# mosure/bevy_gaussian_splatting

Measured on NVIDIA H100. Metric: rendered Msplats/sec @1080p, 6M-gaussian cloud, higher is better.
Workload: dtype f32 (f16-packed inputs)

## Files before the change

bevy_gaussian_splatting_b200/csrc/project.cu:

```cuda
#include "project_math.cuh"
#include "launch.cuh"

namespace bgs {

__constant__ float c_shc[16] = {
    0.28209479177387814f, -0.4886025119029199f, 0.4886025119029199f, -0.4886025119029199f,
    1.0925484305920792f, -1.0925484305920792f, 0.31539156525252005f, -1.0925484305920792f,
    0.5462742152960396f, -0.5900435899266435f, 2.890611442640554f, -0.4570457994644658f,
    0.3731763325901154f, -0.4570457994644658f, 1.445305721320277f, -0.5900435899266435f};

__device__ __forceinline__ void normalize3(const float a[3], float out[3]) {
    const float inv = rsqrtf((a[0] * a[0] + a[1] * a[1]) + a[2] * a[2]);
    out[0] = a[0] * inv; out[1] = a[1] * inv; out[2] = a[2] * inv;
}
__device__ __forceinline__ float dot3(const float a[3], const float b[3]) {
    return (a[0] * b[0] + a[1] * b[1]) + a[2] * b[2];
}
__device__ __forceinline__ float srgb_to_linear(float v) {
    if (v <= 0.04045f) return v * (1.0f / 12.92f);
    return __powf((v + 0.055f) * (1.0f / 1.055f), 2.4f);
}
__device__ __forceinline__ uint32_t pack_bbox(float lo, float hi) {
    return (uint32_t)(int)lo | ((uint32_t)(int)hi << 16);
}
constexpr uint32_t BBOX_EMPTY = 1u;

__device__ __forceinline__ void make_bbox(float cx, float cy, float hx, float hy, int Wi, int Hi,
                                          uint32_t& bx, uint32_t& by) {
    bx = BBOX_EMPTY; by = BBOX_EMPTY;
    if (!(hx >= 0.0f) || !(hy >= 0.0f) || !(cx == cx) || !(cy == cy)) return;
    const float sx = hx * 1.0e-3f + 1.0e-2f, sy = hy * 1.0e-3f + 1.0e-2f;
    float x0 = ceilf((cx - hx) - (0.5f + sx));
    float x1 = floorf((cx + hx) - (0.5f - sx));
    float y0 = ceilf((cy - hy) - (0.5f + sy));
    float y1 = floorf((cy + hy) - (0.5f - sy));
    if (!(x0 <= x1) || !(y0 <= y1)) return;
    x0 = fmaxf(x0, 0.0f); y0 = fmaxf(y0, 0.0f);
    x1 = fminf(x1, (float)(Wi - 1)); y1 = fminf(y1, (float)(Hi - 1));
    if (!(x0 <= x1) || !(y0 <= y1)) return;
    bx = pack_bbox(x0, x1); by = pack_bbox(y0, y1);
}

__device__ __forceinline__ void cp_async16(uint4* dst_shared, const uint4* src) {
    asm volatile("cp.async.cg.shared.global [%0], [%1], 16;" ::"r"((uint32_t)__cvta_generic_to_shared(dst_shared)), "l"(src)
                 : "memory");
}
__device__ __forceinline__ void cp_async_commit() { asm volatile("cp.async.commit_group;" ::: "memory"); }
template <int N>
__device__ __forceinline__ void cp_async_wait() { asm volatile("cp.async.wait_group %0;" ::"n"(N) : "memory"); }

template <int CH>
__device__ __forceinline__ int stage_slot(int p, int g) {
    static_assert(CH % 8 == 0 || CH == 4, "blocks of 4 or a multiple of 8 chunks");
    if constexpr (CH == 4) return p ^ ((g >> 1) & 3);
    else return p ^ (g & 7);
}

template <int CH, int NP>
__device__ __forceinline__ void gather_blocks(const uint4* __restrict__ blocks, uint32_t id, uint32_t n_valid,
                                              uint4* stage, int lane) {
    static_assert(32 % NP == 0 && NP <= CH, "NP lanes per block");
#pragma unroll
    for (int k = 0; k < NP; ++k) {
        const int g = (32 * k + lane) / NP, p = lane % NP;
        const uint32_t gid = __shfl_sync(0xFFFFFFFFu, id, g);
        if ((uint32_t)g < n_valid) cp_async16(stage + g * CH + stage_slot<CH>(p, g), blocks + (size_t)gid * CH + p);
    }
}

template <bool F16, uint32_t D>
struct Attr;
template <uint32_t D>
struct Attr<false, D> {
    static constexpr CloudLayout L = CloudLayout::F32;
    static constexpr int CH = chunks(L, D), GEO = 4;
    __device__ static float4 load(const uint4* stage, int g, float* sh, float q[4], float so[4], bool need_sh, uint32_t&) {
        auto piece = [&](int p) {
            const uint4 v = stage[g * CH + stage_slot<CH>(p, g)];
            return make_float4(__uint_as_float(v.x), __uint_as_float(v.y), __uint_as_float(v.z), __uint_as_float(v.w));
        };
        const float4 p = piece(POS_CHUNK), r = piece(SECOND_CHUNK), s = piece(SO_CHUNK);
        q[0] = r.x; q[1] = r.y; q[2] = r.z; q[3] = r.w;
        so[0] = s.x; so[1] = s.y; so[2] = s.z; so[3] = s.w;
        if (need_sh) {
#pragma unroll
            for (int i = 0; i < (int)sh_chunks(L, D); ++i) {
                const float4 v = piece(sh_first(L) + i);
                sh[4 * i] = v.x; sh[4 * i + 1] = v.y; sh[4 * i + 2] = v.z; sh[4 * i + 3] = v.w;
            }
        }
        return p;
    }
};
template <uint32_t D>
struct Attr<true, D> {
    static constexpr CloudLayout L = CloudLayout::F16;
    static constexpr int CH = chunks(L, D), GEO = 2;
    static constexpr int FULL = (int)sh_floats(D) / 8;
    __device__ static float4 load(const uint4* stage, int g, float* sh, float q[4], float so[4], bool need_sh,
                                  uint32_t& op_bits) {
        auto piece = [&](int p) { return stage[g * CH + stage_slot<CH>(p, g)]; };
        const uint4 pw = piece(POS_CHUNK), w = piece(SECOND_CHUNK);
        op_bits = w.w & 0xFFFFu;
        second_lanes(w.x, w.y, q);
        second_lanes(w.z, w.w, so);
        if (need_sh) {
#pragma unroll
            for (int i = 0; i < FULL; ++i) {
                const uint4 v = piece(sh_first(L) + i);
                sh[8 * i] = half_lo(v.x); sh[8 * i + 1] = half_hi(v.x); sh[8 * i + 2] = half_lo(v.y); sh[8 * i + 3] = half_hi(v.y);
                sh[8 * i + 4] = half_lo(v.z); sh[8 * i + 5] = half_hi(v.z); sh[8 * i + 6] = half_lo(v.w); sh[8 * i + 7] = half_hi(v.w);
            }
            if constexpr (sh_floats(D) % 8 != 0) {
                const uint4 v = piece(sh_first(L) + FULL);
                sh[8 * FULL] = half_lo(v.x); sh[8 * FULL + 1] = half_hi(v.x);
                sh[8 * FULL + 2] = half_lo(v.y); sh[8 * FULL + 3] = half_hi(v.y);
            }
        }
        return make_float4(__uint_as_float(pw.x), __uint_as_float(pw.y), __uint_as_float(pw.z), __uint_as_float(pw.w));
    }
};

template <CloudLayout L, uint32_t D>
__device__ __forceinline__ void repack_chunk(const CloudPlanes<const uint4>& planes, uint32_t n, uint4* __restrict__ blocks,
                                             const uint4* __restrict__ tt) {
    constexpr uint32_t CH = chunks(L, D);
    const size_t i = (size_t)blockIdx.x * blockDim.x + threadIdx.x;
    if (i >= (size_t)n * CH) return;
    const uint4* src = planes.unit<L, D>((uint32_t)(i % CH), i / CH, tt);
    blocks[i] = src ? __ldg(src) : make_uint4(0u, 0u, 0u, 0u);
}
template <CloudLayout L, uint32_t D>
__global__ void repack_kernel(CloudPlanes<const uint4> planes, uint32_t n, uint4* __restrict__ blocks) {
    repack_chunk<L, D>(planes, n, blocks, nullptr);
}
__global__ void repack_4d_kernel(CloudPlanes<const uint4> planes, uint32_t n, uint4* __restrict__ blocks,
                                 const uint4* __restrict__ tt) {
    repack_chunk<CloudLayout::F32x4D, SH_DEGREE_MAX>(planes, n, blocks, tt);
}
void launch_repack(CloudLayout layout, uint32_t sh_degree, const void* sh, const void* rot, const void* so, const void* tt,
                   uint32_t n, CloudView cloud, cudaStream_t stream) {
    const CloudPlanes<const uint4> planes{reinterpret_cast<const uint4*>(cloud.pos), static_cast<const uint4*>(sh),
                                          static_cast<const uint4*>(rot), static_cast<const uint4*>(so)};
    const uint32_t grid = (uint32_t)(((size_t)n * cloud.chunks + 255) / 256);
    with_layout_degree(layout, sh_degree, [&](auto L, auto D) {
        if constexpr (is_4d(decltype(L)::value))
            repack_4d_kernel<<<grid, 256, 0, stream>>>(planes, n, cloud.blocks, static_cast<const uint4*>(tt));
        else
            repack_kernel<decltype(L)::value, decltype(D)::value><<<grid, 256, 0, stream>>>(planes, n, cloud.blocks);
    });
}

__global__ void depth_range_kernel(const float4* __restrict__ pos, uint32_t n, const uint32_t* __restrict__ sorted_payload,
                                   const uint32_t* __restrict__ slot_ids ,
                                   FrameCounters* __restrict__ ctr, FrameConsts fc) {
    if (threadIdx.x != 0 || blockIdx.x != 0 || n < 2u) return;
    const uint32_t n_vis = ctr->n_vis, n_sorted = ctr->n_sort;
    auto id_at = [&](uint32_t i) { const uint32_t p = sorted_payload[i]; return slot_ids ? slot_ids[p] : p; };
    uint32_t first, last;
    if (n_sorted == n) {
        first = id_at(1u); last = id_at(n - 1u);
    } else {
        const uint32_t cmin = 0xFFFFFFFFu - ctr->culled_min_inv, cmax = ctr->culled_max_p1 - 1u;
        first = n_vis >= 2u ? id_at(1u) : cmin;
        last = (n - n_vis) >= 1u ? cmax : id_at(n - 1u);
    }
    auto dist = [&](uint32_t id) {
        const float4 p = pos[id];
        float pw[4];
        mat4_point(fc.model, p.x, p.y, p.z, pw);
        return sqrtf(cam_dist2(fc, pw));
    };
    ctr->depth_min = dist(last);
    ctr->depth_max = dist(first);
}

__device__ __forceinline__ float adaptive_cutoff(float opacity) {
    const float a = 9.0f + 2.0f * det_ln(opacity);
    return sqrtf(a > 0.000001f ? a : 0.000001f);
}
__global__ void cutoff_table_kernel(float* __restrict__ tab) {
    const uint32_t h = blockIdx.x * blockDim.x + threadIdx.x;
    if (h < 65536u) tab[h] = adaptive_cutoff(__half2float(__ushort_as_half((unsigned short)h)));
}
void launch_cutoff_table(float* tab, cudaStream_t stream) { cutoff_table_kernel<<<256, 256, 0, stream>>>(tab); }

template <bool F16>
__device__ __forceinline__ float splat_cutoff(const FrameConsts& fc, float opacity, const float* __restrict__ cutoff_tab,
                                              uint32_t op_bits) {
    if (!fc.adaptive) return 3.0f;
    if constexpr (F16) return __ldg(cutoff_tab + op_bits);
    else return adaptive_cutoff(opacity);
}

__device__ __forceinline__ void rotation_rows(const float q[4], float Rm[3][3]) {
    const float qr = q[0], x = q[1], y = q[2], z = q[3];
    Rm[0][0] = 1.0f - 2.0f * (y * y + z * z);
    Rm[1][0] = 2.0f * (x * y - qr * z);
    Rm[2][0] = 2.0f * (x * z + qr * y);
    Rm[0][1] = 2.0f * (x * y + qr * z);
    Rm[1][1] = 1.0f - 2.0f * (x * x + z * z);
    Rm[2][1] = 2.0f * (y * z - qr * x);
    Rm[0][2] = 2.0f * (x * z - qr * y);
    Rm[1][2] = 2.0f * (y * z + qr * x);
    Rm[2][2] = 1.0f - 2.0f * (x * x + y * y);
}

__device__ __forceinline__ void sigma3d(const FrameConsts& fc, const float A[3][3], const float Rm[3][3], const float sc[3],
                                        const float q[4], const float so[4], float c3[6]) {
    if (fc.cov_pre) {
        c3[0] = q[0]; c3[1] = q[1]; c3[2] = q[2]; c3[3] = q[3]; c3[4] = so[0]; c3[5] = so[1];
        return;
    }
    float M[3][3], Sg[3][3], X[3][3], TS[3][3];
#pragma unroll
    for (int i = 0; i < 3; ++i)
#pragma unroll
        for (int j = 0; j < 3; ++j) M[i][j] = sc[i] * Rm[i][j];
#pragma unroll
    for (int i = 0; i < 3; ++i)
#pragma unroll
        for (int j = 0; j < 3; ++j) Sg[i][j] = (M[0][i] * M[0][j] + M[1][i] * M[1][j]) + M[2][i] * M[2][j];
    const float mn = fminf(fminf(fminf(fabsf(Sg[0][0]), fabsf(Sg[0][1])), fminf(fabsf(Sg[0][2]), fabsf(Sg[1][1]))),
                           fminf(fabsf(Sg[1][2]), fabsf(Sg[2][2])));
    const float mx = fmaxf(fmaxf(fmaxf(fabsf(Sg[0][0]), fabsf(Sg[0][1])), fmaxf(fabsf(Sg[0][2]), fabsf(Sg[1][1]))),
                           fmaxf(fabsf(Sg[1][2]), fabsf(Sg[2][2])));
    if (fc.model_identity && mn > 0.0f && mx < __uint_as_float(0x7F800000u) && Sg[0][0] == Sg[0][0] &&
        Sg[0][1] == Sg[0][1] && Sg[0][2] == Sg[0][2] && Sg[1][1] == Sg[1][1] && Sg[1][2] == Sg[1][2] && Sg[2][2] == Sg[2][2]) {
#pragma unroll
        for (int i = 0; i < 3; ++i)
#pragma unroll
            for (int j = 0; j < 3; ++j) TS[i][j] = Sg[i][j];
    } else {
#pragma unroll
        for (int i = 0; i < 3; ++i)
#pragma unroll
            for (int j = 0; j < 3; ++j) X[i][j] = (A[i][0] * Sg[0][j] + A[i][1] * Sg[1][j]) + A[i][2] * Sg[2][j];
#pragma unroll
        for (int i = 0; i < 3; ++i)
#pragma unroll
            for (int j = 0; j < 3; ++j) TS[i][j] = (X[i][0] * A[j][0] + X[i][1] * A[j][1]) + X[i][2] * A[j][2];
    }
    c3[0] = TS[0][0]; c3[1] = TS[1][0]; c3[2] = TS[2][0]; c3[3] = TS[1][1]; c3[4] = TS[2][1]; c3[5] = TS[2][2];
}

struct Cov2d {
    float a, b, c, det, mid, term, l1;
};
__device__ __forceinline__ Cov2d cov2d(const FrameConsts& fc, const float pw[3], const float c3[6]) {
    const float Vrk[3][3] = {{c3[0], c3[1], c3[2]}, {c3[1], c3[3], c3[4]}, {c3[2], c3[4], c3[5]}};
    float tv[4];
    mat4_point(fc.view_from_world, pw[0], pw[1], pw[2], tv);
    const float fx = fc.p00 * fc.W, fy = fc.p11 * fc.H;
    const float sz = 1.0f / (tv[2] * tv[2]);
    const float J00 = fx / tv[2], J20 = -(fx * tv[0]) * sz;
    const float J11 = -fy / tv[2], J21 = (fy * tv[1]) * sz;
    float Tm[3][2];
#pragma unroll
    for (int i = 0; i < 3; ++i) {
        const float v0 = fc.view_from_world[i * 4 + 0], v1 = fc.view_from_world[i * 4 + 1],
                    v2 = fc.view_from_world[i * 4 + 2];
        Tm[i][0] = v0 * J00 + v2 * J20;
        Tm[i][1] = v1 * J11 + v2 * J21;
    }
    float Y[3][2];
#pragma unroll
    for (int i = 0; i < 3; ++i)
#pragma unroll
        for (int b = 0; b < 2; ++b) Y[i][b] = (Vrk[i][0] * Tm[0][b] + Vrk[i][1] * Tm[1][b]) + Vrk[i][2] * Tm[2][b];
    Cov2d v;
    v.a = ((Tm[0][0] * Y[0][0] + Tm[1][0] * Y[1][0]) + Tm[2][0] * Y[2][0]) + 0.3f;
    v.b = (Tm[0][1] * Y[0][0] + Tm[1][1] * Y[1][0]) + Tm[2][1] * Y[2][0];
    v.c = ((Tm[0][1] * Y[0][1] + Tm[1][1] * Y[1][1]) + Tm[2][1] * Y[2][1]) + 0.3f;
    v.det = v.a * v.c - v.b * v.b;
    v.mid = 0.5f * (v.a + v.c);
    v.term = sqrtf(fmaxf(0.0f, v.mid * v.mid - v.det));
    v.l1 = v.mid + v.term;
    return v;
}

__device__ __forceinline__ void aabb_record(const FrameConsts& fc, const Cov2d& v, float cutoff, SplatRec& rec) {
    const float l2 = fmaxf(v.mid - v.term, 0.0f);
    const float Rq = cutoff * fmaxf(sqrtf(v.l1), sqrtf(l2));
    const float dinv = 1.0f / v.det;
    rec.ux = v.c * dinv; rec.uy = -v.b * dinv; rec.vx = v.a * dinv; rec.vy = Rq;
    const float h = 0.5f * Rq;
    make_bbox(rec.cx, rec.cy, h, h, fc.Wi, fc.Hi, rec.bx, rec.by);
}

__device__ __forceinline__ void obb_record(const FrameConsts& fc, const Cov2d& v, float cutoff, SplatRec& rec) {
    const float a = v.a, b = v.b, c = v.c;
    const float aa = (a - c) * (a - c);
    const float bb = sqrtf(aa + (4.0f * b) * b);
// ... 139 lines not shown
    mat4_dir(fc.view_from_world, Ln[0], Ln[1], Ln[2], wn);
    const float l = sqrtf(((wn[0] * wn[0] + wn[1] * wn[1]) + wn[2] * wn[2]) + wn[3] * wn[3]);
#pragma unroll
    for (int cc = 0; cc < 3; ++cc) rgb[cc] = 0.5f * (wn[cc] / l + 1.0f);
}

__device__ __forceinline__ void position_colour(const FrameConsts& fc, const float pw[3], float rgb[3]) {
#pragma unroll
    for (int cc = 0; cc < 3; ++cc) rgb[cc] = (pw[cc] - fc.aabb_min[cc]) / (fc.aabb_max[cc] - fc.aabb_min[cc]);
}

constexpr float FRAC_PI_3_F = 1.0471975512f;
constexpr float PI_2_F = 6.28318530718f;

__device__ __forceinline__ void hsv_to_rgb(float h, float s, float v, float rgb[3]) {
    const float hk = h / FRAC_PI_3_F, vs = v * s;
    const float base[3] = {5.0f, 3.0f, 1.0f};
#pragma unroll
    for (int cc = 0; cc < 3; ++cc) {
        const float x = base[cc] + hk;
        const float k = x - 6.0f * truncf(x / 6.0f);
        rgb[cc] = v - vs * fmaxf(0.0f, fminf(k, fminf(4.0f - k, 1.0f)));
    }
}

__device__ __forceinline__ float det_atan2(float yf, float xf) {
    if (yf != yf || xf != xf) return __uint_as_float(0x7FC00000u);
    const double ay = fabs((double)yf), ax = fabs((double)xf);
    const bool steep = ay > ax;
    double t;
    if (ax == ay) t = ax == 0.0 ? 0.0 : 1.0;
    else t = steep ? __ddiv_rn(ax, ay) : __ddiv_rn(ay, ax);
    double base = 0.0, u = t;
    if (t > 0.41421356237309503) { base = 0.7853981633974483; u = __ddiv_rn(__dsub_rn(t, 1.0), __dadd_rn(t, 1.0)); }
    const double z = __dmul_rn(u, u);
    double p = -1.0 / 43.0;
#pragma unroll
    for (int k = 20; k >= 0; --k) p = __dadd_rn(__dmul_rn(p, z), (k & 1 ? -1.0 : 1.0) / (double)(2 * k + 1));
    double r = __dadd_rn(base, __dmul_rn(u, p));
    if (steep) r = __dsub_rn(1.5707963267948966, r);
    if (__float_as_uint(xf) >> 31) r = __dsub_rn(3.141592653589793, r);
    if (__float_as_uint(yf) >> 31) r = -r;
    return (float)r;
}

__device__ __forceinline__ void class_colour(const ModeConsts& mc, float vis, float rgb[3]) {
    if (vis < 2.0f) return;
    const float hue = ((vis - 2.0f) / (float)mc.num_classes) * 6.283185307f;
    float h[3];
    hsv_to_rgb(hue, 1.0f, 1.0f, h);
#pragma unroll
    for (int cc = 0; cc < 3; ++cc) rgb[cc] = rgb[cc] * (1.0f - 0.5f) + h[cc] * 0.5f;
}

__device__ __forceinline__ void flow_colour_from(const FrameConsts& fc, const ModeConsts& mc, const float pw[3],
                                                 const float pw_prev[3], float rgb[3]) {
    float c[4], cp[4];
    mat4_point(fc.clip_from_world, pw[0], pw[1], pw[2], c);
    mat4_point(mc.prev_clip_from_world, pw_prev[0], pw_prev[1], pw_prev[2], cp);
    const float mvx = (c[0] / c[3] - cp[0] / cp[3]) * 0.5f;
    const float mvy = (c[1] / c[3] - cp[1] / cp[3]) * -0.5f;
    const float fx = mvx / mc.delta_time, fy = mvy / mc.delta_time;
    const float radius = sqrtf(fx * fx + fy * fy);
    float angle = det_atan2(fy, fx);
    if (angle < 0.0f) angle = angle + PI_2_F;
    hsv_to_rgb(angle, fminf(fmaxf(radius, 0.0f), 1.0f), 1.0f, rgb);
}
__device__ __forceinline__ void flow_colour(const FrameConsts& fc, const ModeConsts& mc, const float pw[3], float rgb[3]) {
    flow_colour_from(fc, mc, pw, pw, rgb);
}

__device__ __forceinline__ void highlight_selected(SplatRec& rec, float drgb[3], float nrgb[3]) {
    rec.r = 0.3f; rec.g = 1.0f; rec.b = 0.1f; rec.op = 1.0f;
    drgb[0] = nrgb[0] = 0.3f; drgb[1] = nrgb[1] = 1.0f; drgb[2] = nrgb[2] = 0.1f;
}

__device__ __forceinline__ void store_rec(SplatRec* __restrict__ dst, const SplatRec& rec) {
    float4* out = reinterpret_cast<float4*>(dst);
    out[0] = make_float4(rec.cx, rec.cy, rec.ux, rec.uy);
    out[1] = make_float4(rec.vx, rec.vy, __uint_as_float(rec.bx), __uint_as_float(rec.by));
    out[2] = make_float4(rec.r, rec.g, rec.b, rec.op);
}

template <bool F16, uint32_t D, bool MODES2>
__device__ __forceinline__ void project_one(const FrameConsts& fc, const FrameCounters* __restrict__ ctr, uint32_t r,
                                            float4 p4, const float q[4], const float so[4], const float* sh,
                                            const float* __restrict__ cutoff_tab, uint32_t op_bits,
                                            SplatRec* __restrict__ recs, float4* __restrict__ extra,
                                            float4* __restrict__ aux, const ModeConsts& mc, bool no_source = false) {
    SplatRec rec;
    rec.ux = 0.f; rec.uy = 0.f; rec.vx = 0.f; rec.vy = 0.f;
    rec.bx = BBOX_EMPTY; rec.by = BBOX_EMPTY;
    rec.r = 0.f; rec.g = 0.f; rec.b = 0.f;
    float pw[4], ndc[2];
    mat4_point(fc.model, p4.x, p4.y, p4.z, pw);
    const bool visible = in_frustum(fc, pw, ndc);
    const float hw = 0.5f * fc.W, hh = 0.5f * fc.H;
    rec.cx = ndc[0] * hw + hw;
    rec.cy = hh - ndc[1] * hh;
    const float opacity = so[3];
    rec.op = opacity * fc.global_opacity;
    if (visible && !no_source && !(fc.draw_mode == BGS_DRAW_SELECTED && p4.w < 0.5f)) {
        const float cutoff = splat_cutoff<F16>(fc, opacity, cutoff_tab, op_bits);
        float A[3][3], Rm[3][3];
#pragma unroll
        for (int rr = 0; rr < 3; ++rr)
#pragma unroll
            for (int cc = 0; cc < 3; ++cc) A[rr][cc] = fc.model[cc * 4 + rr];
        rotation_rows(q, Rm);
        const float sc[3] = {so[0] * fc.global_scale, so[1] * fc.global_scale, so[2] * fc.global_scale};

        if (fc.gaussian_mode == BGS_GAUSSIAN_3D) {
            float c3[6];
            sigma3d(fc, A, Rm, sc, q, so, c3);
            const Cov2d v = cov2d(fc, pw, c3);
            if (fc.aabb) aabb_record(fc, v, cutoff, rec);
            else obb_record(fc, v, cutoff, rec);
        } else {
            surfel_record(fc, A, Rm, sc, pw, cutoff, r, extra, rec);
        }

        const uint32_t mode = fc.rasterize_mode;
        float rgb[3] = {0.f, 0.f, 0.f}, drgb[3] = {0.f, 0.f, 0.f}, nrgb[3] = {0.f, 0.f, 0.f};
        if constexpr (MODES2) {
            if (mode == BGS_RASTERIZE_CLASSIFICATION) {
                sh_colour<D>(fc, A, pw, sh, rgb);
                class_colour(mc, p4.w, rgb);
            } else {
                flow_colour(fc, mc, pw, rgb);
            }
            rec.r = rgb[0]; rec.g = rgb[1]; rec.b = rgb[2];
        } else {
            if (mode == BGS_RASTERIZE_COLOR) sh_colour<D>(fc, A, pw, sh, rgb);
            if (mode == BGS_RASTERIZE_POSITION) position_colour(fc, pw, rgb);
            if (mode == BGS_RASTERIZE_DEPTH || fc.aux) depth_colour(fc, ctr, pw, drgb);
            if (mode == BGS_RASTERIZE_NORMAL || fc.aux) normal_colour(fc, A, Rm, sc, nrgb);
            const bool depth = mode == BGS_RASTERIZE_DEPTH, normal = mode == BGS_RASTERIZE_NORMAL;
            rec.r = depth ? drgb[0] : normal ? nrgb[0] : rgb[0];
            rec.g = depth ? drgb[1] : normal ? nrgb[1] : rgb[1];
            rec.b = depth ? drgb[2] : normal ? nrgb[2] : rgb[2];
        }
        if (fc.draw_mode == BGS_DRAW_HIGHLIGHT_SELECTED && p4.w > 0.5f) highlight_selected(rec, drgb, nrgb);
        if (fc.aux && aux != nullptr) {
            aux[(size_t)r * 2] = make_float4(drgb[0], drgb[1], drgb[2], 0.0f);
            aux[(size_t)r * 2 + 1] = make_float4(nrgb[0], nrgb[1], nrgb[2], 0.0f);
        }
    }
    store_rec(recs + r, rec);
}

constexpr int PROJ_THREADS = 128, PROJ_WARPS = PROJ_THREADS / 32, PROJ_MIN_CTAS = 4;

template <bool F16, uint32_t D, bool MODES2>
__device__ __forceinline__ void project_groups(const void* __restrict__ blocks, const uint32_t* __restrict__ index_list,
                                               int by_slot, const FrameCounters* __restrict__ ctr, const FrameConsts& fc,
                                               bool need_sh, SplatRec* __restrict__ recs, float4* __restrict__ extra,
                                               const float* __restrict__ cutoff_tab, float4* __restrict__ aux,
                                               const ModeConsts& mc) {
    using A = Attr<F16, D>;
    constexpr int CH = A::CH;
    __shared__ __align__(16) uint4 s_stages[PROJ_WARPS][32 * CH];
    const int lane = threadIdx.x & 31;
    uint4* const stage = s_stages[threadIdx.x >> 5];
    const uint32_t n_vis = ctr->n_vis, stride = gridDim.x * PROJ_THREADS;
    auto list_id = [&](uint32_t r) {
        return r < n_vis ? (by_slot ? __ldg(index_list + r) : __ldg(index_list + (n_vis - 1u - r))) : 0u;
    };
    auto gather = [&](uint32_t r0, uint32_t id) {
        const uint32_t n_valid = r0 < n_vis ? n_vis - r0 : 0u;
        const uint4* b = reinterpret_cast<const uint4*>(blocks);
        if (need_sh) gather_blocks<CH, CH>(b, id, n_valid, stage, lane);
        else gather_blocks<CH, A::GEO>(b, id, n_valid, stage, lane);
        cp_async_commit();
    };
    uint32_t r0 = (blockIdx.x * PROJ_WARPS + (threadIdx.x >> 5)) * 32u;
    gather(r0, list_id(r0 + lane));
    uint32_t id_next = list_id(r0 + stride + lane);
    for (; r0 < n_vis; r0 += stride) {
        cp_async_wait<0>();
        __syncwarp();
        const uint32_t r = r0 + lane;
        float sh[sh_floats(D)], q[4], so[4];
        uint32_t op_bits = 0u;
        float4 p4 = make_float4(0.f, 0.f, 0.f, 0.f);
        if (r < n_vis) p4 = A::load(stage, lane, sh, q, so, need_sh, op_bits);
        __syncwarp();
        gather(r0 + stride, id_next);
        id_next = list_id(r0 + 2u * stride + lane);
        if (r < n_vis) project_one<F16, D, MODES2>(fc, ctr, r, p4, q, so, sh, cutoff_tab, op_bits, recs, extra, aux, mc);
    }
}

template <bool F16, uint32_t D>
__global__ void __launch_bounds__(PROJ_THREADS, PROJ_MIN_CTAS)
project_kernel(const void* __restrict__ blocks, const uint32_t* __restrict__ index_list, int by_slot,
               const FrameCounters* __restrict__ ctr, FrameConsts fc, SplatRec* __restrict__ recs,
               float4* __restrict__ extra , const float* __restrict__ cutoff_tab,
               float4* __restrict__ aux ) {
    project_groups<F16, D, false>(blocks, index_list, by_slot, ctr, fc, fc.rasterize_mode == BGS_RASTERIZE_COLOR, recs, extra,
                               cutoff_tab, aux, ModeConsts{});
}

template <bool F16, uint32_t D>
__global__ void __launch_bounds__(PROJ_THREADS, PROJ_MIN_CTAS)
project_modes_kernel(const void* __restrict__ blocks, const uint32_t* __restrict__ index_list, int by_slot,
                     const FrameCounters* __restrict__ ctr, FrameConsts fc, ModeConsts mc, SplatRec* __restrict__ recs,
                     float4* __restrict__ extra, const float* __restrict__ cutoff_tab) {
    project_groups<F16, D, true>(blocks, index_list, by_slot, ctr, fc, fc.rasterize_mode == BGS_RASTERIZE_CLASSIFICATION, recs,
                              extra, cutoff_tab, nullptr, mc);
}

template <int CH, int NP>
__device__ __forceinline__ void gather_block_ptrs(const uint4* block , uint4* stage, int lane) {
#pragma unroll
    for (int k = 0; k < NP; ++k) {
        const int g = (32 * k + lane) / NP, p = lane % NP;
        const uint4* src = reinterpret_cast<const uint4*>(
            __shfl_sync(0xFFFFFFFFu, (unsigned long long)reinterpret_cast<uintptr_t>(block), g));
        if (src) cp_async16(stage + g * CH + stage_slot<CH>(p, g), src + p);
    }
}

template <bool F16, uint32_t D, bool MODES2>
__device__ __forceinline__ void project_scene_groups(const SceneTable& tab, uint32_t group, const uint32_t* __restrict__ slot_ids,
                                                     const FrameCounters* __restrict__ ctr, bool need_sh,
                                                     SplatRec* __restrict__ recs, float4* __restrict__ extra,
                                                     const float* __restrict__ cutoff_tab, const ModeConsts& mc) {
    using A = Attr<F16, D>;
    constexpr int CH = A::CH;
    __shared__ __align__(16) uint4 s_stages[PROJ_WARPS][32 * CH];
    const int lane = threadIdx.x & 31;
    uint4* const stage = s_stages[threadIdx.x >> 5];
    const uint32_t n_vis = ctr->n_vis, stride = gridDim.x * PROJ_THREADS;
    constexpr uint32_t NONE = 0xFFFFFFFFu;
    auto list_id = [&](uint32_t r) { return r < n_vis ? __ldg(slot_ids + r) : NONE; };
    auto block_of = [&](uint32_t g) -> const uint4* {
        if (g == NONE) return nullptr;
        const SceneSeg& s = tab.seg[tab.find(g)];
        if (s.group != group) return nullptr;
        return static_cast<const uint4*>(s.blocks) + (size_t)(g - s.offset) * CH;
    };
    auto gather = [&](uint32_t g) {
        const uint4* block = block_of(g);
        if (need_sh) gather_block_ptrs<CH, CH>(block, stage, lane);
        else gather_block_ptrs<CH, A::GEO>(block, stage, lane);
        cp_async_commit();
    };
    uint32_t r0 = (blockIdx.x * PROJ_WARPS + (threadIdx.x >> 5)) * 32u;
    uint32_t g_cur = list_id(r0 + lane);
    gather(g_cur);
    uint32_t g_next = list_id(r0 + stride + lane);
    for (; r0 < n_vis; r0 += stride) {
        cp_async_wait<0>();
        __syncwarp();
        const uint32_t r = r0 + lane;
        const uint32_t j = g_cur == NONE ? 0u : tab.find(g_cur);
        const bool mine = g_cur != NONE && tab.seg[j].group == group;
        float sh[sh_floats(D)], q[4], so[4];
        uint32_t op_bits = 0u;
        float4 p4 = make_float4(0.f, 0.f, 0.f, 0.f);
        if (mine) p4 = A::load(stage, lane, sh, q, so, need_sh, op_bits);
        __syncwarp();
        gather(g_next);
        g_cur = g_next;
        g_next = list_id(r0 + 2u * stride + lane);
        if (mine)
            project_one<F16, D, MODES2>(tab.seg[j].fc, ctr, r, p4, q, so, sh, cutoff_tab, op_bits, recs, extra, nullptr, mc,
                                        MODES2 && tab.seg[j].fc.rasterize_mode == BGS_RASTERIZE_VELOCITY);
    }
}

template <bool F16, uint32_t D>
constexpr int scene_min_ctas() { return !F16 && D >= 2 ? 3 : PROJ_MIN_CTAS; }

template <bool F16, uint32_t D>
__global__ void __launch_bounds__(PROJ_THREADS, scene_min_ctas<F16, D>())
project_scene_kernel(SceneTable tab, uint32_t group, const uint32_t* __restrict__ slot_ids, const FrameCounters* __restrict__ ctr,
                     SplatRec* __restrict__ recs, float4* __restrict__ extra, const float* __restrict__ cutoff_tab) {
    project_scene_groups<F16, D, false>(tab, group, slot_ids, ctr, tab.seg[0].fc.rasterize_mode == BGS_RASTERIZE_COLOR, recs,
                                        extra, cutoff_tab, ModeConsts{});
}
template <bool F16, uint32_t D>
__global__ void __launch_bounds__(PROJ_THREADS, scene_min_ctas<F16, D>())
// ... 258 lines not shown
                                                         recs, depths);
}

__global__ void __launch_bounds__(PROJ_THREADS, PROJ_MIN_CTAS)
project_4d_scene_kernel(SceneTable tab, SceneTimes times, ModeConsts mc, const uint32_t* __restrict__ slot_ids,
                        const FrameCounters* __restrict__ ctr, SplatRec* __restrict__ recs,
                        float* __restrict__ depths ) {
    __shared__ __align__(16) uint4 s_stages[PROJ_WARPS][32 * GEO4];
    const int lane = threadIdx.x & 31;
    uint4* const stage = s_stages[threadIdx.x >> 5];
    const uint32_t n_vis = ctr->n_vis, stride = gridDim.x * PROJ_THREADS;
    constexpr uint32_t NONE = 0xFFFFFFFFu;
    auto list_id = [&](uint32_t r) { return r < n_vis ? __ldg(slot_ids + r) : NONE; };
    auto block_of = [&](uint32_t g) -> const uint4* {
        if (g == NONE) return nullptr;
        const SceneSeg& s = tab.seg[tab.find(g)];
        if (s.group != PROJECT_GROUP_4D) return nullptr;
        return static_cast<const uint4*>(s.blocks) + (size_t)(g - s.offset) * CH4;
    };
    auto gather = [&](uint32_t g) {
        gather_block_ptrs<GEO4, GEO4>(block_of(g), stage, lane);
        cp_async_commit();
    };
    uint32_t r0 = (blockIdx.x * PROJ_WARPS + (threadIdx.x >> 5)) * 32u;
    uint32_t g_cur = list_id(r0 + lane);
    gather(g_cur);
    uint32_t g_next = list_id(r0 + stride + lane);
    for (; r0 < n_vis; r0 += stride) {
        cp_async_wait<0>();
        __syncwarp();
        const uint32_t r = r0 + lane;
        const uint32_t j = g_cur == NONE ? 0u : tab.find(g_cur);
        const bool mine = g_cur != NONE && tab.seg[j].group == PROJECT_GROUP_4D;
        auto piece = [&](int p) {
            const uint4 v = stage[lane * GEO4 + (p ^ (lane & 7))];
            return make_float4(__uint_as_float(v.x), __uint_as_float(v.y), __uint_as_float(v.z), __uint_as_float(v.w));
        };
        const float4 p4 = piece(POS_CHUNK), a = piece(SECOND_CHUNK), b = piece(ROT_R_CHUNK), c = piece(SO_4D_CHUNK),
                     d = piece(TT_CHUNK);
        __syncwarp();
        const uint32_t g_mine = g_cur;
        gather(g_next);
        g_cur = g_next;
        g_next = list_id(r0 + 2u * stride + lane);
        if (mine) {
            const SceneSeg& s = tab.seg[j];
            const float ql[4] = {a.x, a.y, a.z, a.w}, qr[4] = {b.x, b.y, b.z, b.w}, so[4] = {c.x, c.y, c.z, c.w},
                        tt[4] = {d.x, d.y, d.z, d.w};
            const uint4* sh = static_cast<const uint4*>(s.blocks) + (size_t)(g_mine - s.offset) * CH4 + sh_first(CloudLayout::F32x4D);
            project_one_4d(s.fc, mc, times.t[j], ctr, r, p4, ql, qr, so, tt, sh, recs, depths);
        }
    }
}
static_assert(sizeof(SceneTable) + sizeof(SceneTimes) + sizeof(ModeConsts) + 4 * sizeof(void*) + 16 <= 32764,
              "project_4d_scene_kernel's parameters exceed the sm_90 limit");

void launch_project_4d_scene(const SceneTable& tab, const SceneTimes& times, const uint32_t* slot_ids, const FrameCounters* ctr,
                             const ModeConsts& mc, SplatRec* recs, float* depths, uint32_t n_hint, int sm_count,
                             cudaStream_t stream) {
    uint32_t grid = (n_hint + PROJ_THREADS - 1) / PROJ_THREADS;
    if (grid > (uint32_t)(PROJ_MIN_CTAS * sm_count)) grid = (uint32_t)(PROJ_MIN_CTAS * sm_count);
    if (grid < 1u) grid = 1u;
    project_4d_scene_kernel<<<grid, PROJ_THREADS, 0, stream>>>(tab, times, mc, slot_ids, ctr, recs, depths);
}

void launch_depth_range(const float4* pos, uint32_t n, const uint32_t* sorted_payload, const uint32_t* slot_ids,
                        FrameCounters* ctr, const FrameConsts& fc, cudaStream_t stream) {
    depth_range_kernel<<<1, 32, 0, stream>>>(pos, n, sorted_payload, slot_ids, ctr, fc);
}

void launch_project(CloudLayout layout, uint32_t sh_degree, const void* blocks, const uint32_t* index_list, int by_slot, const FrameCounters* ctr,
                    const FrameConsts& fc, SplatRec* recs, float4* extra, uint32_t n_hint, int sm_count,
                    const float* cutoff_tab, float4* aux, const ModeConsts* modes, cudaStream_t stream) {
    uint32_t grid = (n_hint + PROJ_THREADS - 1) / PROJ_THREADS;
    if (grid > (uint32_t)(PROJ_MIN_CTAS * sm_count)) grid = (uint32_t)(PROJ_MIN_CTAS * sm_count);
    if (grid < 1u) grid = 1u;
    with_layout_degree(layout, sh_degree, [&](auto L, auto Dt) {
        constexpr CloudLayout Lv = decltype(L)::value;
        constexpr uint32_t D = decltype(Dt)::value;
        if constexpr (!is_4d(Lv)) {
            if (modes)
                project_modes_kernel<is_f16(Lv), D><<<grid, PROJ_THREADS, 0, stream>>>(blocks, index_list, by_slot, ctr, fc, *modes,
                                                                                      recs, extra, cutoff_tab);
            else
                project_kernel<is_f16(Lv), D><<<grid, PROJ_THREADS, 0, stream>>>(blocks, index_list, by_slot, ctr, fc, recs, extra,
                                                                                cutoff_tab, aux);
        }
    });
}

}
```

bevy_gaussian_splatting_b200/csrc/project_math.cuh:

```cuda
#pragma once
#include "common.cuh"

namespace bgs {

__device__ __forceinline__ void mat4_point(const float* m, float x, float y, float z, float out[4]) {
#pragma unroll
    for (int r = 0; r < 4; ++r) out[r] = ((m[0 + r] * x + m[4 + r] * y) + m[8 + r] * z) + m[12 + r];
}
__device__ __forceinline__ void mat4_dir(const float* m, float x, float y, float z, float out[4]) {
#pragma unroll
    for (int r = 0; r < 4; ++r) out[r] = (m[0 + r] * x + m[4 + r] * y) + m[8 + r] * z;
}

__device__ __forceinline__ void keygen_world_pos(const FrameConsts& c, float4 p, float pw[4]) {
    if (c.model_identity && (fabsf(p.x) + fabsf(p.y)) + fabsf(p.z) < __uint_as_float(0x7F800000u)) {
        pw[0] = p.x; pw[1] = p.y; pw[2] = p.z; pw[3] = 1.0f;
    } else {
        mat4_point(c.model, p.x, p.y, p.z, pw);
    }
}

__device__ __forceinline__ void world_to_clip(const FrameConsts& c, const float pw[3], float out[4]) {
    float cl[4];
    mat4_point(c.clip_from_world, pw[0], pw[1], pw[2], cl);
    const float den = cl[3] + 0.000000001f;
#pragma unroll
    for (int i = 0; i < 4; ++i) out[i] = cl[i] / den;
}

__device__ __forceinline__ bool in_frustum(const FrameConsts& c, const float pw[3], float ndc[2]) {
    float h[4];
    world_to_clip(c, pw, h);
    const float nx = h[0], ny = h[1], nz = h[2];
    ndc[0] = nx; ndc[1] = ny;
    return fabsf(nx) < 1.1f && fabsf(ny) < 1.1f && fabsf(nz - 0.5f) < 0.5f;
}

__device__ __forceinline__ float splat_depth(const FrameConsts& c, const float pw[3]) {
    float h[4];
    world_to_clip(c, pw, h);
    return h[2] / h[3];
}

__device__ __forceinline__ bool in_frustum_fast(const FrameConsts& c, const float pw[3]) {
    float cl[4];
    mat4_point(c.clip_from_world, pw[0], pw[1], pw[2], cl);
    const float den = cl[3] + 0.000000001f;
    float rc;
    asm("rcp.approx.ftz.f32 %0, %1;" : "=f"(rc) : "f"(den));
    const float ax = fabsf(cl[0] * rc), ay = fabsf(cl[1] * rc), z = cl[2] * rc;
    const float ad = fabsf(den);
    const bool sure_in = ax < 1.0999f && ay < 1.0999f && z > 1e-6f && z < 0.9999f;
    const bool sure_out = ax > 1.1001f || ay > 1.1001f || z < -1e-6f || z > 1.0001f;
    const bool den_ok = ad > 1e-30f && ad < 1e30f;
    if (den_ok && (sure_in || sure_out)) return sure_in;
    float ndc[2];
    return in_frustum(c, pw, ndc);
}

__device__ __forceinline__ float cam_dist2(const FrameConsts& c, const float pw[3]) {
    const float dx = pw[0] - c.cam[0], dy = pw[1] - c.cam[1], dz = pw[2] - c.cam[2];
    return (dx * dx + dy * dy) + dz * dz;
}

__device__ __forceinline__ uint32_t depth_key(const FrameConsts& c, bool visible, float d2) {
    uint32_t key = 0xFFFFFFFFu;
    if (visible) key = 0xFFFFFFFFu - __float_as_uint(d2);
    return key >> c.key_shift;
}

__device__ __forceinline__ float det_ln(float xf) {
    if (xf != xf) return xf;
    if (xf < 0.0f) return __uint_as_float(0x7FC00000u);
    if (xf == 0.0f) return __uint_as_float(0xFF800000u);
    if (xf == __uint_as_float(0x7F800000u)) return xf;
    const double x = (double)xf;
    unsigned long long bits = (unsigned long long)__double_as_longlong(x);
    int e = (int)((bits >> 52) & 0x7FFull) - 1023;
    bits = (bits & 0x000FFFFFFFFFFFFFull) | 0x3FF0000000000000ull;
    double m = __longlong_as_double((long long)bits);
    if (m > 1.4142135623730951) { m = __dmul_rn(m, 0.5); e += 1; }
    const double s = __ddiv_rn(__dsub_rn(m, 1.0), __dadd_rn(m, 1.0));
    const double z = __dmul_rn(s, s);
    double p = 1.0 / 23.0;
    p = __dadd_rn(__dmul_rn(p, z), 1.0 / 21.0);
    p = __dadd_rn(__dmul_rn(p, z), 1.0 / 19.0);
    p = __dadd_rn(__dmul_rn(p, z), 1.0 / 17.0);
    p = __dadd_rn(__dmul_rn(p, z), 1.0 / 15.0);
    p = __dadd_rn(__dmul_rn(p, z), 1.0 / 13.0);
    p = __dadd_rn(__dmul_rn(p, z), 1.0 / 11.0);
    p = __dadd_rn(__dmul_rn(p, z), 1.0 / 9.0);
    p = __dadd_rn(__dmul_rn(p, z), 1.0 / 7.0);
    p = __dadd_rn(__dmul_rn(p, z), 1.0 / 5.0);
    p = __dadd_rn(__dmul_rn(p, z), 1.0 / 3.0);
    p = __dadd_rn(__dmul_rn(p, z), 1.0);
    const double r = __dadd_rn(__dmul_rn((double)e, 0.6931471805599453), __dmul_rn(2.0, __dmul_rn(s, p)));
    return (float)r;
}

// ... 36 lines not shown
```

Measured before the change: 18040.

## Add specialized plain-frame projection kernel with split gather and skipped frustum test

Adds a PLAIN template path and a dedicated project_plain_kernel, selected when the frame uses 3D gaussians, colour mode, OBB, no aux, no precomputed covariance and no highlight. On that path the world position skips the model matrix when it is identity, the frustum test is dropped because slot-indexed entries are assumed already visible, mode branches are compiled out, and a new gather routine issues all cp.async chunks with precomputed shared addresses. The aim is to cut per-splat branching, the frustum math and address arithmetic in the common case. It relies on by_slot lists being pre-culled, and the extra kernel instantiation adds code size.

```diff
diff --git a/bevy_gaussian_splatting_b200/csrc/project.cu b/bevy_gaussian_splatting_b200/csrc/project.cu
--- a/bevy_gaussian_splatting_b200/csrc/project.cu
+++ b/bevy_gaussian_splatting_b200/csrc/project.cu
@@ -41,9 +41,11 @@
     bx = pack_bbox(x0, x1); by = pack_bbox(y0, y1);
 }
 
+__device__ __forceinline__ void cp_async16(uint32_t dst_shared , const uint4* src) {
+    asm volatile("cp.async.cg.shared.global [%0], [%1], 16;" ::"r"(dst_shared), "l"(src) : "memory");
+}
 __device__ __forceinline__ void cp_async16(uint4* dst_shared, const uint4* src) {
-    asm volatile("cp.async.cg.shared.global [%0], [%1], 16;" ::"r"((uint32_t)__cvta_generic_to_shared(dst_shared)), "l"(src)
-                 : "memory");
+    cp_async16((uint32_t)__cvta_generic_to_shared(dst_shared), src);
 }
 __device__ __forceinline__ void cp_async_commit() { asm volatile("cp.async.commit_group;" ::: "memory"); }
 template <int N>
@@ -65,6 +67,22 @@
         const int g = (32 * k + lane) / NP, p = lane % NP;
         const uint32_t gid = __shfl_sync(0xFFFFFFFFu, id, g);
         if ((uint32_t)g < n_valid) cp_async16(stage + g * CH + stage_slot<CH>(p, g), blocks + (size_t)gid * CH + p);
+    }
+}
+
+template <int CH>
+__device__ __forceinline__ void gather_blocks_split(const uint4* __restrict__ blocks, uint32_t id, uint32_t n_valid,
+                                                    uint4* stage, int lane) {
+    constexpr int M = 32 / CH;
+    const uint32_t stage_addr = (uint32_t)__cvta_generic_to_shared(stage);
+    const uint32_t u0 = (uint32_t)((lane / CH) * CH + stage_slot<CH>(lane % CH, lane / CH));
+    const uint4* src = blocks + lane % CH;
+#pragma unroll
+    for (int k = 0; k < CH; ++k) {
+        const int g = k * M + lane / CH;
+        const uint32_t gid = __shfl_sync(0xFFFFFFFFu, id, g);
+        const uint32_t unit = (u0 ^ (uint32_t)stage_slot<CH>(0, k * M)) + 32u * k;
+        if ((uint32_t)g < n_valid) cp_async16(stage_addr + unit * 16u, src + (size_t)gid * CH);
     }
 }
 
@@ -206,9 +224,10 @@
     Rm[2][2] = 1.0f - 2.0f * (x * x + y * y);
 }
 
+template <bool PLAIN>
 __device__ __forceinline__ void sigma3d(const FrameConsts& fc, const float A[3][3], const float Rm[3][3], const float sc[3],
                                         const float q[4], const float so[4], float c3[6]) {
-    if (fc.cov_pre) {
+    if (!PLAIN && fc.cov_pre) {
         c3[0] = q[0]; c3[1] = q[1]; c3[2] = q[2]; c3[3] = q[3]; c3[4] = so[0]; c3[5] = so[1];
         return;
     }
@@ -514,19 +533,29 @@
     out[2] = make_float4(rec.r, rec.g, rec.b, rec.op);
 }
 
-template <bool F16, uint32_t D, bool MODES2>
+template <bool F16, uint32_t D, bool MODES2, bool PLAIN = false>
 __device__ __forceinline__ void project_one(const FrameConsts& fc, const FrameCounters* __restrict__ ctr, uint32_t r,
                                             float4 p4, const float q[4], const float so[4], const float* sh,
                                             const float* __restrict__ cutoff_tab, uint32_t op_bits,
                                             SplatRec* __restrict__ recs, float4* __restrict__ extra,
                                             float4* __restrict__ aux, const ModeConsts& mc, bool no_source = false) {
+    static_assert(!(PLAIN && MODES2), "the plain frame's colour source is Color");
     SplatRec rec;
     rec.ux = 0.f; rec.uy = 0.f; rec.vx = 0.f; rec.vy = 0.f;
     rec.bx = BBOX_EMPTY; rec.by = BBOX_EMPTY;
     rec.r = 0.f; rec.g = 0.f; rec.b = 0.f;
     float pw[4], ndc[2];
-    mat4_point(fc.model, p4.x, p4.y, p4.z, pw);
-    const bool visible = in_frustum(fc, pw, ndc);
+    bool visible;
+    if constexpr (PLAIN) {
+        projection_world_pos(fc, p4, pw);
+        float h[4];
+        world_to_clip(fc, pw, h);
+        ndc[0] = h[0]; ndc[1] = h[1];
+        visible = true;
+    } else {
+        mat4_point(fc.model, p4.x, p4.y, p4.z, pw);
+        visible = in_frustum(fc, pw, ndc);
+    }
     const float hw = 0.5f * fc.W, hh = 0.5f * fc.H;
     rec.cx = ndc[0] * hw + hw;
     rec.cy = hh - ndc[1] * hh;
@@ -542,11 +571,11 @@
         rotation_rows(q, Rm);
         const float sc[3] = {so[0] * fc.global_scale, so[1] * fc.global_scale, so[2] * fc.global_scale};
 
-        if (fc.gaussian_mode == BGS_GAUSSIAN_3D) {
+        if (PLAIN || fc.gaussian_mode == BGS_GAUSSIAN_3D) {
             float c3[6];
-            sigma3d(fc, A, Rm, sc, q, so, c3);
+            sigma3d<PLAIN>(fc, A, Rm, sc, q, so, c3);
             const Cov2d v = cov2d(fc, pw, c3);
-            if (fc.aabb) aabb_record(fc, v, cutoff, rec);
+            if (!PLAIN && fc.aabb) aabb_record(fc, v, cutoff, rec);
             else obb_record(fc, v, cutoff, rec);
         } else {
             surfel_record(fc, A, Rm, sc, pw, cutoff, r, extra, rec);
@@ -554,7 +583,10 @@
 
         const uint32_t mode = fc.rasterize_mode;
         float rgb[3] = {0.f, 0.f, 0.f}, drgb[3] = {0.f, 0.f, 0.f}, nrgb[3] = {0.f, 0.f, 0.f};
-        if constexpr (MODES2) {
+        if constexpr (PLAIN) {
+            sh_colour<D>(fc, A, pw, sh, rgb);
+            rec.r = rgb[0]; rec.g = rgb[1]; rec.b = rgb[2];
+        } else if constexpr (MODES2) {
             if (mode == BGS_RASTERIZE_CLASSIFICATION) {
                 sh_colour<D>(fc, A, pw, sh, rgb);
                 class_colour(mc, p4.w, rgb);
@@ -572,8 +604,8 @@
             rec.g = depth ? drgb[1] : normal ? nrgb[1] : rgb[1];
             rec.b = depth ? drgb[2] : normal ? nrgb[2] : rgb[2];
         }
-        if (fc.draw_mode == BGS_DRAW_HIGHLIGHT_SELECTED && p4.w > 0.5f) highlight_selected(rec, drgb, nrgb);
-        if (fc.aux && aux != nullptr) {
+        if (!PLAIN && fc.draw_mode == BGS_DRAW_HIGHLIGHT_SELECTED && p4.w > 0.5f) highlight_selected(rec, drgb, nrgb);
+        if (!PLAIN && fc.aux && aux != nullptr) {
             aux[(size_t)r * 2] = make_float4(drgb[0], drgb[1], drgb[2], 0.0f);
             aux[(size_t)r * 2 + 1] = make_float4(nrgb[0], nrgb[1], nrgb[2], 0.0f);
         }
@@ -583,7 +615,7 @@
 
 constexpr int PROJ_THREADS = 128, PROJ_WARPS = PROJ_THREADS / 32, PROJ_MIN_CTAS = 4;
 
-template <bool F16, uint32_t D, bool MODES2>
+template <bool F16, uint32_t D, bool MODES2, bool PLAIN = false>
 __device__ __forceinline__ void project_groups(const void* __restrict__ blocks, const uint32_t* __restrict__ index_list,
                                                int by_slot, const FrameCounters* __restrict__ ctr, const FrameConsts& fc,
                                                bool need_sh, SplatRec* __restrict__ recs, float4* __restrict__ extra,
@@ -601,7 +633,8 @@
     auto gather = [&](uint32_t r0, uint32_t id) {
         const uint32_t n_valid = r0 < n_vis ? n_vis - r0 : 0u;
         const uint4* b = reinterpret_cast<const uint4*>(blocks);
-        if (need_sh) gather_blocks<CH, CH>(b, id, n_valid, stage, lane);
+        if constexpr (PLAIN) gather_blocks_split<CH>(b, id, n_valid, stage, lane);
+        else if (need_sh) gather_blocks<CH, CH>(b, id, n_valid, stage, lane);
         else gather_blocks<CH, A::GEO>(b, id, n_valid, stage, lane);
         cp_async_commit();
     };
@@ -619,7 +652,7 @@
         __syncwarp();
         gather(r0 + stride, id_next);
         id_next = list_id(r0 + 2u * stride + lane);
-        if (r < n_vis) project_one<F16, D, MODES2>(fc, ctr, r, p4, q, so, sh, cutoff_tab, op_bits, recs, extra, aux, mc);
+        if (r < n_vis) project_one<F16, D, MODES2, PLAIN>(fc, ctr, r, p4, q, so, sh, cutoff_tab, op_bits, recs, extra, aux, mc);
     }
 }
 
@@ -631,6 +664,17 @@
                float4* __restrict__ aux ) {
     project_groups<F16, D, false>(blocks, index_list, by_slot, ctr, fc, fc.rasterize_mode == BGS_RASTERIZE_COLOR, recs, extra,
                                cutoff_tab, aux, ModeConsts{});
+}
+
+template <bool F16, uint32_t D>
+__global__ void __launch_bounds__(PROJ_THREADS, PROJ_MIN_CTAS)
+project_plain_kernel(const void* __restrict__ blocks, const uint32_t* __restrict__ slot_ids, const FrameCounters* __restrict__ ctr,
+                     FrameConsts fc, SplatRec* __restrict__ recs, const float* __restrict__ cutoff_tab) {
+    project_groups<F16, D, false, true>(blocks, slot_ids, 1, ctr, fc, true, recs, nullptr, cutoff_tab, nullptr, ModeConsts{});
+}
+static bool plain_frame(const FrameConsts& fc, int by_slot) {
+    return by_slot && fc.gaussian_mode == BGS_GAUSSIAN_3D && !fc.aabb && fc.rasterize_mode == BGS_RASTERIZE_COLOR && !fc.aux &&
+           !fc.cov_pre && fc.draw_mode != BGS_DRAW_HIGHLIGHT_SELECTED;
 }
 
 template <bool F16, uint32_t D>
@@ -1055,6 +1099,9 @@
             if (modes)
                 project_modes_kernel<is_f16(Lv), D><<<grid, PROJ_THREADS, 0, stream>>>(blocks, index_list, by_slot, ctr, fc, *modes,
                                                                                       recs, extra, cutoff_tab);
+            else if (plain_frame(fc, by_slot))
+                project_plain_kernel<is_f16(Lv), D><<<grid, PROJ_THREADS, 0, stream>>>(blocks, index_list, ctr, fc, recs,
+                                                                                            cutoff_tab);
             else
                 project_kernel<is_f16(Lv), D><<<grid, PROJ_THREADS, 0, stream>>>(blocks, index_list, by_slot, ctr, fc, recs, extra,
                                                                                 cutoff_tab, aux);
diff --git a/bevy_gaussian_splatting_b200/csrc/project_math.cuh b/bevy_gaussian_splatting_b200/csrc/project_math.cuh
--- a/bevy_gaussian_splatting_b200/csrc/project_math.cuh
+++ b/bevy_gaussian_splatting_b200/csrc/project_math.cuh
@@ -15,6 +15,14 @@
 __device__ __forceinline__ void keygen_world_pos(const FrameConsts& c, float4 p, float pw[4]) {
     if (c.model_identity && (fabsf(p.x) + fabsf(p.y)) + fabsf(p.z) < __uint_as_float(0x7F800000u)) {
         pw[0] = p.x; pw[1] = p.y; pw[2] = p.z; pw[3] = 1.0f;
+    } else {
+        mat4_point(c.model, p.x, p.y, p.z, pw);
+    }
+}
+
+__device__ __forceinline__ void projection_world_pos(const FrameConsts& c, float4 p, float pw[4]) {
+    if (c.model_identity && (fabsf(p.x) + fabsf(p.y)) + fabsf(p.z) < __uint_as_float(0x7F800000u)) {
+        pw[0] = p.x + 0.0f; pw[1] = p.y + 0.0f; pw[2] = p.z + 0.0f; pw[3] = 1.0f;
     } else {
         mat4_point(c.model, p.x, p.y, p.z, pw);
     }
```

After: 18300, median of 6. 1.01x the previous value.
